# pengsongyou/openscene

Hardware: AMD Instinct MI355X
Metric: active voxels/sec MinkUNet18A fwd+bwd @2cm ScanNet; per-point query ms (higher is better)
Workload: dtype f32 (bf16x6 split-precision MFMA, fp32 accumulate); 1 GPU; ScanNet distillation step (configs[2]): MinkUNet18A, 768-d head, 1 synthetic S100k scene/GPU (100999 voxels on rank 0, 2 cm), training-mode BN; timed = coordinate+kernel maps, forward, cosine loss, backward, gradient all-reduce, Adam step; arch=MinkUNet18A, feature_dim=768, voxels_rank0=100999, parallelism=dp1

## Files before the change

### openscene_amd/csrc/bn.hip

```cpp
#include "common.h"
#include "epilogue.h"

namespace osn {

constexpr int CR_COLS = 64;
constexpr int CR_RL = 16;
constexpr int CR_MAX_BLOCKS = 512;

constexpr int BN_MAX_SRC = 3;
struct GySrc {
    const float* p[BN_MAX_SRC];
    int64_t ld[BN_MAX_SRC];
    int n;
};

__device__ inline float4 gy_load(const GySrc& s, int64_t r, int col) {
    float4 g = *reinterpret_cast<const float4*>(s.p[0] + r * s.ld[0] + col);
#pragma unroll
    for (int i = 1; i < BN_MAX_SRC; ++i)
        if (i < s.n) {
            const float4 v = *reinterpret_cast<const float4*>(s.p[i] + r * s.ld[i] + col);
            g.x += v.x; g.y += v.y; g.z += v.z; g.w += v.w;
        }
    return g;
}


struct ColReducePlan {
    int n_rb;
    int n_cg;
    int rows_per_block;
};

static ColReducePlan plan_colreduce(int64_t n, int c) {
    ColReducePlan p;
    p.n_cg = int(cdiv(c, CR_COLS));
    int64_t rb = cdiv(n, 4 * CR_RL);
    if (rb > CR_MAX_BLOCKS) rb = CR_MAX_BLOCKS;
    if (rb < 1) rb = 1;
    p.rows_per_block = int(cdiv(cdiv(n, rb), CR_RL) * CR_RL);
    p.n_rb = int(cdiv(n, p.rows_per_block));
    if (p.n_rb < 1) p.n_rb = 1;
    return p;
}

template <int MODE>
__global__ __launch_bounds__(256) void col_reduce_kernel(const float* __restrict__ x, const float* __restrict__ y,
                                                         const GySrc gy, const float* __restrict__ mean,
                                                         const float* __restrict__ var, float eps, int relu, int64_t n,
                                                         int c, int rows_per_block, double* __restrict__ partial,
                                                         const float* __restrict__ gamma, const float* __restrict__ beta) {
    __shared__ double red[2][CR_RL][CR_COLS];
    const int tid = threadIdx.x;
    const int cl = tid & 15, rl = tid >> 4;
    const int col = blockIdx.y * CR_COLS + cl * 4;
    const bool on = col < c;
    const int64_t r0 = int64_t(blockIdx.x) * rows_per_block;
    const int64_t r1 = min(n, r0 + rows_per_block);
    double s1[4] = {0, 0, 0, 0}, s2[4] = {0, 0, 0, 0};
    float4 mu = make_float4(0, 0, 0, 0), is = make_float4(0, 0, 0, 0);
    float4 ga = make_float4(0, 0, 0, 0), be = make_float4(0, 0, 0, 0);
    const bool from_x = MODE == 1 && relu && !y;
    if (MODE == 1 && on) {
        mu = *reinterpret_cast<const float4*>(mean + col);
        const float4 v = *reinterpret_cast<const float4*>(var + col);
        is = make_float4(bn_is(v.x, eps), bn_is(v.y, eps), bn_is(v.z, eps), bn_is(v.w, eps));
        if (from_x) {
            ga = *reinterpret_cast<const float4*>(gamma + col);
            be = *reinterpret_cast<const float4*>(beta + col);
        }
    }
    if (on) {
        for (int64_t r = r0 + rl; r < r1; r += CR_RL) {
            const float4 xv = *reinterpret_cast<const float4*>(x + r * c + col);
            if (MODE == 0) {
                s1[0] += xv.x; s1[1] += xv.y; s1[2] += xv.z; s1[3] += xv.w;
                s2[0] += double(xv.x) * xv.x; s2[1] += double(xv.y) * xv.y;
                s2[2] += double(xv.z) * xv.z; s2[3] += double(xv.w) * xv.w;
            } else {
                float4 g = gy_load(gy, r, col);
                if (from_x) {
                    g.x = bn_val(xv.x, mu.x, is.x, ga.x, be.x) > 0.f ? g.x : 0.f;
                    g.y = bn_val(xv.y, mu.y, is.y, ga.y, be.y) > 0.f ? g.y : 0.f;
                    g.z = bn_val(xv.z, mu.z, is.z, ga.z, be.z) > 0.f ? g.z : 0.f;
                    g.w = bn_val(xv.w, mu.w, is.w, ga.w, be.w) > 0.f ? g.w : 0.f;
                } else if (relu) {
                    const float4 yv = *reinterpret_cast<const float4*>(y + r * c + col);
                    g.x = yv.x > 0.f ? g.x : 0.f; g.y = yv.y > 0.f ? g.y : 0.f;
                    g.z = yv.z > 0.f ? g.z : 0.f; g.w = yv.w > 0.f ? g.w : 0.f;
                }
                s1[0] += g.x; s1[1] += g.y; s1[2] += g.z; s1[3] += g.w;
                s2[0] += double(g.x) * ((xv.x - mu.x) * is.x); s2[1] += double(g.y) * ((xv.y - mu.y) * is.y);
                s2[2] += double(g.z) * ((xv.z - mu.z) * is.z); s2[3] += double(g.w) * ((xv.w - mu.w) * is.w);
            }
        }
    }
#pragma unroll
    for (int j = 0; j < 4; ++j) {
        red[0][rl][cl * 4 + j] = s1[j];
        red[1][rl][cl * 4 + j] = s2[j];
    }
    __syncthreads();
    if (tid < 2 * CR_COLS) {
        const int which = tid / CR_COLS, cc = tid % CR_COLS;
        double s = 0;
#pragma unroll
        for (int r = 0; r < CR_RL; ++r) s += red[which][r][cc];
        const int gc = blockIdx.y * CR_COLS + cc;
        if (gc < c) partial[(int64_t(blockIdx.x) * 2 + which) * c + gc] = s;
    }
}

constexpr int FIN_COLS = 16, FIN_PARTS = 64;

constexpr int FIN_ITERS = CR_MAX_BLOCKS / FIN_PARTS;

__device__ inline void finalize_sums(const double* __restrict__ partial, int n_rb, int c, double& s1, double& s2,
                                     int& col) {
    __shared__ double red[2][FIN_PARTS][FIN_COLS];
    const int cl = threadIdx.x & (FIN_COLS - 1), part = threadIdx.x / FIN_COLS;
    col = blockIdx.x * FIN_COLS + cl;
    double va[FIN_ITERS], vb[FIN_ITERS];
    const int cc = col < c ? col : 0;
#pragma unroll
    for (int i = 0; i < FIN_ITERS; ++i) {
        const int blk = part + FIN_PARTS * i;
        const int bc = blk < n_rb ? blk : 0;
        va[i] = partial[(int64_t(bc) * 2 + 0) * c + cc];
        vb[i] = partial[(int64_t(bc) * 2 + 1) * c + cc];
    }
    double a = 0, b = 0;
#pragma unroll
    for (int i = 0; i < FIN_ITERS; ++i) {
        const bool on = col < c && part + FIN_PARTS * i < n_rb;
        a += on ? va[i] : 0.0;
        b += on ? vb[i] : 0.0;
    }
    red[0][part][cl] = a;
    red[1][part][cl] = b;
    __syncthreads();
    double t1 = 0, t2 = 0;
    if (part < 8) {
#pragma unroll
        for (int q = 0; q < 8; ++q) { t1 += red[0][part * 8 + q][cl]; t2 += red[1][part * 8 + q][cl]; }
    }
    __syncthreads();
    if (part < 8) {
        red[0][part][cl] = t1;
        red[1][part][cl] = t2;
    }
    __syncthreads();
    s1 = 0; s2 = 0;
    if (part == 0) {
#pragma unroll
        for (int q = 0; q < 8; ++q) { s1 += red[0][q][cl]; s2 += red[1][q][cl]; }
    }
}

__global__ __launch_bounds__(FIN_COLS * FIN_PARTS) void bn_stats_finalize_kernel(
    const double* __restrict__ partial, int n_rb, int64_t n, int c, float* __restrict__ mean, float* __restrict__ var,
    float* __restrict__ running_mean, float* __restrict__ running_var, float momentum) {
    double s1, s2;
    int j;
    finalize_sums(partial, n_rb, c, s1, s2, j);
    if (threadIdx.x >= FIN_COLS || j >= c) return;
    const double m = s1 / double(n);
    double v = s2 / double(n) - m * m;
    if (v < 0) v = 0;
    mean[j] = float(m);
    var[j] = float(v);
    if (running_mean) running_mean[j] = (1.f - momentum) * running_mean[j] + momentum * float(m);
    if (running_var) {
        const double unb = n > 1 ? v * double(n) / double(n - 1) : v;
        running_var[j] = (1.f - momentum) * running_var[j] + momentum * float(unb);
    }
}

__global__ __launch_bounds__(FIN_COLS * FIN_PARTS) void bn_bwd_finalize_kernel(const double* __restrict__ partial,
                                                                              int n_rb, int c,
                                                                              float* __restrict__ sum_g,
                                                                              float* __restrict__ sum_gx) {
    double s1, s2;
    int j;
    finalize_sums(partial, n_rb, c, s1, s2, j);
    if (threadIdx.x >= FIN_COLS || j >= c) return;
    sum_g[j] = float(s1);
    sum_gx[j] = float(s2);
}

__device__ inline float4 ld4(const float* p) { return *reinterpret_cast<const float4*>(p); }


__global__ __launch_bounds__(256) void bn_apply_kernel(const float* __restrict__ x, const float* __restrict__ mean,
                                                       const float* __restrict__ var, const float* __restrict__ gamma,
                                                       const float* __restrict__ beta, float eps,
                                                       const float* __restrict__ residual, int relu,
                                                       float* __restrict__ y, float* __restrict__ y2, int64_t ld2,
                                                       int64_t total4, int c4) {
    for (int64_t e = int64_t(blockIdx.x) * blockDim.x + threadIdx.x; e < total4; e += int64_t(gridDim.x) * blockDim.x) {
        const int col = int(e % c4) * 4;
        const float4 xv = ld4(x + e * 4), mu = ld4(mean + col), vv = ld4(var + col), ga = ld4(gamma + col),
                     be = ld4(beta + col);
        float4 o;
        o.x = bn_val(xv.x, mu.x, bn_is(vv.x, eps), ga.x, be.x);
        o.y = bn_val(xv.y, mu.y, bn_is(vv.y, eps), ga.y, be.y);
        o.z = bn_val(xv.z, mu.z, bn_is(vv.z, eps), ga.z, be.z);
        o.w = bn_val(xv.w, mu.w, bn_is(vv.w, eps), ga.w, be.w);
        if (residual) {
            const float4 rv = ld4(residual + e * 4);
            o.x += rv.x; o.y += rv.y; o.z += rv.z; o.w += rv.w;
        }
        if (relu) {
            o.x = bn_relu(o.x); o.y = bn_relu(o.y); o.z = bn_relu(o.z); o.w = bn_relu(o.w);
        }
        *reinterpret_cast<float4*>(y + e * 4) = o;
        if (y2) *reinterpret_cast<float4*>(y2 + (e / c4) * ld2 + col) = o;
    }
}

__global__ __launch_bounds__(256) void bn_bwd_apply_kernel(const float* __restrict__ x, const float* __restrict__ y,
                                                           const GySrc gy, const float* __restrict__ mean,
                                                           const float* __restrict__ var, const float* __restrict__ gamma,
                                                           float eps, int relu, int training,
                                                           const float* __restrict__ sum_g,
                                                           const float* __restrict__ sum_gx, float inv_n,
                                                           float* __restrict__ gx, float* __restrict__ gres,
                                                           int64_t total4, int c4, const float* __restrict__ beta) {
    const bool from_x = relu && !y;
    for (int64_t e = int64_t(blockIdx.x) * blockDim.x + threadIdx.x; e < total4; e += int64_t(gridDim.x) * blockDim.x) {
        const int col = int(e % c4) * 4;
        float4 g = gy_load(gy, e / c4, col);
        const float4 vv = ld4(var + col), ga = ld4(gamma + col);
        const float4 is = make_float4(bn_is(vv.x, eps), bn_is(vv.y, eps), bn_is(vv.z, eps), bn_is(vv.w, eps));
        float4 xv = make_float4(0, 0, 0, 0), mu = make_float4(0, 0, 0, 0);
        if (training || from_x) { xv = ld4(x + e * 4); mu = ld4(mean + col); }
        if (from_x) {
            const float4 be = ld4(beta + col);
            g.x = bn_val(xv.x, mu.x, is.x, ga.x, be.x) > 0.f ? g.x : 0.f;
            g.y = bn_val(xv.y, mu.y, is.y, ga.y, be.y) > 0.f ? g.y : 0.f;
            g.z = bn_val(xv.z, mu.z, is.z, ga.z, be.z) > 0.f ? g.z : 0.f;
            g.w = bn_val(xv.w, mu.w, is.w, ga.w, be.w) > 0.f ? g.w : 0.f;
        } else if (relu) {
            const float4 yv = ld4(y + e * 4);
            g.x = yv.x > 0.f ? g.x : 0.f; g.y = yv.y > 0.f ? g.y : 0.f;
            g.z = yv.z > 0.f ? g.z : 0.f; g.w = yv.w > 0.f ? g.w : 0.f;
        }
        if (gres) *reinterpret_cast<float4*>(gres + e * 4) = g;
        float4 o;
        if (training) {
            const float4 sg = ld4(sum_g + col), sx = ld4(sum_gx + col);
            o.x = ga.x * is.x * (g.x - sg.x * inv_n - (xv.x - mu.x) * is.x * sx.x * inv_n);
            o.y = ga.y * is.y * (g.y - sg.y * inv_n - (xv.y - mu.y) * is.y * sx.y * inv_n);
            o.z = ga.z * is.z * (g.z - sg.z * inv_n - (xv.z - mu.z) * is.z * sx.z * inv_n);
            o.w = ga.w * is.w * (g.w - sg.w * inv_n - (xv.w - mu.w) * is.w * sx.w * inv_n);
        } else {
            o.x = ga.x * is.x * g.x; o.y = ga.y * is.y * g.y; o.z = ga.z * is.z * g.z; o.w = ga.w * is.w * g.w;
        }
        *reinterpret_cast<float4*>(gx + e * 4) = o;
    }
}

constexpr int SB_THREADS = 1024, SB_RL = 512, SB_PER = 8, SB_COLS = 8;
constexpr int SB_MAX_ROWS = SB_RL * SB_PER;

__device__ inline double sb_wave_sum(double v) {
#pragma unroll
    for (int off = 2; off < 64; off <<= 1) v += __shfl_xor(v, off, 64);
    return v;
}

__device__ inline void sb_block_sums(double (&s)[8], int tid, int cl) {
    __shared__ double red[SB_THREADS / 64][2][8];
    __shared__ double tot[2][8];
#pragma unroll
    for (int q = 0; q < 8; ++q) s[q] = sb_wave_sum(s[q]);
    const int lane = tid & 63, wave = tid >> 6;
    if ((lane >> 1) == 0) {
#pragma unroll
        for (int q = 0; q < 8; ++q) red[wave][cl][q] = s[q];
    }
    __syncthreads();
    if (tid < 16) {
        const int c2 = tid >> 3, q = tid & 7;
        double t = 0;
#pragma unroll
        for (int w = 0; w < SB_THREADS / 64; ++w) t += red[w][c2][q];
        tot[c2][q] = t;
    }
    __syncthreads();
#pragma unroll
    for (int q = 0; q < 8; ++q) s[q] = tot[cl][q];
}

__global__ __launch_bounds__(SB_THREADS) void bn_small_fwd_kernel(const float* __restrict__ x, int n, int c,
                                                                  const float* __restrict__ gamma, const float* __restrict__ beta,
                                                                  float eps, const float* __restrict__ residual, int relu,
                                                                  float momentum, float* __restrict__ mean_out,
                                                                  float* __restrict__ var_out, float* __restrict__ running_mean,
                                                                  float* __restrict__ running_var, float* __restrict__ y,
                                                                  float* __restrict__ y2, int64_t ld2) {
    const int tid = threadIdx.x, cl = tid & 1, rl = tid >> 1;
    const int col = blockIdx.x * SB_COLS + cl * 4;
    const bool con = col < c;
    const int cc = con ? col : 0;
    float4 v[SB_PER];
    double s[8] = {0, 0, 0, 0, 0, 0, 0, 0};
#pragma unroll
    for (int j = 0; j < SB_PER; ++j) {
        const int r = rl + SB_RL * j;
        const bool ok = con && r < n;
        v[j] = ld4(x + int64_t(ok ? r : 0) * c + cc);
        if (ok) {
            s[0] += v[j].x; s[1] += v[j].y; s[2] += v[j].z; s[3] += v[j].w;
            s[4] += double(v[j].x) * v[j].x; s[5] += double(v[j].y) * v[j].y;
            s[6] += double(v[j].z) * v[j].z; s[7] += double(v[j].w) * v[j].w;
        }
    }
    sb_block_sums(s, tid, cl);
    float mu[4], vr[4];
#pragma unroll
    for (int q = 0; q < 4; ++q) {
        const double m = s[q] / double(n);
        double var = s[4 + q] / double(n) - m * m;
        if (var < 0) var = 0;
        mu[q] = float(m);
        vr[q] = float(var);
        if (rl == 0 && con) {
            mean_out[col + q] = mu[q];
            var_out[col + q] = vr[q];
            if (running_mean) running_mean[col + q] = (1.f - momentum) * running_mean[col + q] + momentum * mu[q];
            if (running_var) {
                const double unb = n > 1 ? var * double(n) / double(n - 1) : var;
                running_var[col + q] = (1.f - momentum) * running_var[col + q] + momentum * float(unb);
            }
        }
    }
    if (!con) return;
    const float4 ga = ld4(gamma + col), be = ld4(beta + col);
    const float is0 = bn_is(vr[0], eps), is1 = bn_is(vr[1], eps), is2 = bn_is(vr[2], eps), is3 = bn_is(vr[3], eps);
#pragma unroll
    for (int j = 0; j < SB_PER; ++j) {
        const int r = rl + SB_RL * j;
        if (r >= n) continue;
        float4 o;
        o.x = bn_val(v[j].x, mu[0], is0, ga.x, be.x);
        o.y = bn_val(v[j].y, mu[1], is1, ga.y, be.y);
        o.z = bn_val(v[j].z, mu[2], is2, ga.z, be.z);
        o.w = bn_val(v[j].w, mu[3], is3, ga.w, be.w);
        if (residual) {
            const float4 rv = ld4(residual + int64_t(r) * c + col);
            o.x += rv.x; o.y += rv.y; o.z += rv.z; o.w += rv.w;
        }
        if (relu) {
            o.x = bn_relu(o.x); o.y = bn_relu(o.y); o.z = bn_relu(o.z); o.w = bn_relu(o.w);
        }
        *reinterpret_cast<float4*>(y + int64_t(r) * c + col) = o;
        if (y2) *reinterpret_cast<float4*>(y2 + int64_t(r) * ld2 + col) = o;
    }
}

static int ew_grid(int64_t total4) {
    int64_t g = cdiv(total4, 256);
    if (g > 2048) g = 2048;
    if (g < 1) g = 1;
    return int(g);
}

}

using namespace osn;

extern "C" size_t osn_bn_ws_bytes(int64_t n, int c) {
    (void)n;
    return size_t(CR_MAX_BLOCKS) * 2 * size_t(c) * 8 + 256;
}

extern "C" int osn_bn_stats(const float* x, int64_t n, int c, float* mean, float* var, float* running_mean,
                            float* running_var, float momentum, void* ws, size_t ws_bytes, osn_stream_t stream) {
    hipStream_t st = static_cast<hipStream_t>(stream);
    OSN_REQUIRE(n >= 1 && c >= 4 && (c & 3) == 0, OSN_E_ARG, "osn_bn_stats: need n >= 1 and c %% 4 == 0 (n=%lld c=%d)", (long long)n, c);
    OSN_REQUIRE(x && mean && var && aligned16(x), OSN_E_ARG, "osn_bn_stats: null or unaligned pointer");
    ColReducePlan p = plan_colreduce(n, c);
    const size_t need = size_t(p.n_rb) * 2 * size_t(c) * 8;
    OSN_REQUIRE(ws && ws_bytes >= need, OSN_E_WS, "osn_bn_stats: workspace %zu < %zu", ws_bytes, need);
    double* partial = static_cast<double*>(ws);
    hipLaunchKernelGGL((col_reduce_kernel<0>), dim3(p.n_rb, p.n_cg), dim3(256), 0, st, x, (const float*)nullptr,
                       GySrc{}, (const float*)nullptr, (const float*)nullptr, 0.f, 0, n, c,
                       p.rows_per_block, partial, (const float*)nullptr, (const float*)nullptr);
    hipLaunchKernelGGL(bn_stats_finalize_kernel, dim3(cdiv(c, FIN_COLS)), dim3(FIN_COLS * FIN_PARTS), 0, st, partial, p.n_rb, n, c, mean, var,
                       running_mean, running_var, momentum);
    OSN_LAUNCH_CHECK();
    return OSN_OK;
}

extern "C" int osn_bn_apply2(const float* x, const float* mean, const float* var, const float* gamma, const float* beta,
                             float eps, const float* residual, int relu, float* y, float* y2, int64_t ld2, int64_t n, int c,
                             osn_stream_t stream) {
    hipStream_t st = static_cast<hipStream_t>(stream);
    OSN_REQUIRE(n >= 0 && c >= 4 && (c & 3) == 0, OSN_E_ARG, "osn_bn_apply: need c %% 4 == 0 (c=%d)", c);
    if (n == 0) return OSN_OK;
    OSN_REQUIRE(x && mean && var && gamma && beta && y, OSN_E_ARG, "osn_bn_apply: null pointer");
    OSN_REQUIRE(aligned16(x) && aligned16(y) && aligned16(mean) && aligned16(var) && aligned16(gamma) && aligned16(beta) &&
                    (!residual || aligned16(residual)),
                OSN_E_ARG, "osn_bn_apply: pointers must be 16-byte aligned");
    OSN_REQUIRE(!y2 || (aligned16(y2) && ld2 >= c && (ld2 & 3) == 0), OSN_E_ARG,
                "osn_bn_apply2: the second destination needs a 16-byte aligned pointer and a row stride >= c, %% 4 == 0");
    const int64_t total4 = n * (c / 4);
    hipLaunchKernelGGL(bn_apply_kernel, dim3(ew_grid(total4)), dim3(256), 0, st, x, mean, var, gamma, beta, eps,
                       residual, relu, y, y2, ld2, total4, c / 4);
    OSN_LAUNCH_CHECK();
    return OSN_OK;
}

extern "C" int osn_bn_apply(const float* x, const float* mean, const float* var, const float* gamma, const float* beta,
                            float eps, const float* residual, int relu, float* y, int64_t n, int c,
                            osn_stream_t stream) {
    return osn_bn_apply2(x, mean, var, gamma, beta, eps, residual, relu, y, nullptr, 0, n, c, stream);
}

extern "C" int osn_bn_forward_train2(const float* x, int64_t n, int c, const float* gamma, const float* beta, float eps,
                                     const float* residual, int relu, float momentum, float* mean, float* var,
                                     float* running_mean, float* running_var, float* y, float* y2, int64_t ld2, void* ws,
                                     size_t ws_bytes, osn_stream_t stream) {
    if (n >= 1 && n <= SB_MAX_ROWS && c >= 4 && (c & 3) == 0) {
        hipStream_t st = static_cast<hipStream_t>(stream);
        OSN_REQUIRE(x && mean && var && gamma && beta && y, OSN_E_ARG, "osn_bn_forward_train: null pointer");
        OSN_REQUIRE(aligned16(x) && aligned16(y) && aligned16(gamma) && aligned16(beta) && (!residual || aligned16(residual)),
                    OSN_E_ARG, "osn_bn_forward_train: pointers must be 16-byte aligned");
        OSN_REQUIRE(!y2 || (aligned16(y2) && ld2 >= c && (ld2 & 3) == 0), OSN_E_ARG,
                    "osn_bn_forward_train2: the second destination needs a 16-byte aligned pointer and a row stride >= c, %% 4 == 0");
        hipLaunchKernelGGL(bn_small_fwd_kernel, dim3(unsigned(cdiv(c, SB_COLS))), dim3(SB_THREADS), 0, st, x, int(n), c, gamma,
                           beta, eps, residual, relu, momentum, mean, var, running_mean, running_var, y, y2, ld2);
        OSN_LAUNCH_CHECK();
        return OSN_OK;
    }
    int rc = osn_bn_stats(x, n, c, mean, var, running_mean, running_var, momentum, ws, ws_bytes, stream);
    if (rc) return rc;
    return osn_bn_apply2(x, mean, var, gamma, beta, eps, residual, relu, y, y2, ld2, n, c, stream);
}

extern "C" int osn_bn_forward_train(const float* x, int64_t n, int c, const float* gamma, const float* beta, float eps,
                                    const float* residual, int relu, float momentum, float* mean, float* var,
                                    float* running_mean, float* running_var, float* y, void* ws, size_t ws_bytes,
                                    osn_stream_t stream) {
    return osn_bn_forward_train2(x, n, c, gamma, beta, eps, residual, relu, momentum, mean, var, running_mean, running_var, y,
                                 nullptr, 0, ws, ws_bytes, stream);
}

extern "C" int osn_bn_backward_multi2(const float* x, const float* y, const float* const* gy, const int64_t* gy_ld, int n_gy,
                                      const float* mean, const float* var, const float* gamma, const float* beta, float eps, int relu,
                                     int training, float* gx, float* gres, float* ggamma, float* gbeta, int64_t n, int c,
                                     void* ws, size_t ws_bytes, osn_stream_t stream) {
    hipStream_t st = static_cast<hipStream_t>(stream);
    OSN_REQUIRE(n >= 1 && c >= 4 && (c & 3) == 0, OSN_E_ARG, "osn_bn_backward: need n >= 1 and c %% 4 == 0");
    OSN_REQUIRE(gy && gy_ld && n_gy >= 1 && n_gy <= BN_MAX_SRC, OSN_E_ARG,
                "osn_bn_backward: %d gradient sources (1 .. %d are supported)", n_gy, BN_MAX_SRC);
    OSN_REQUIRE(x && mean && var && gamma && gx && ggamma && gbeta && (!relu || y || beta), OSN_E_ARG,
                "osn_bn_backward: null pointer");
    OSN_REQUIRE(!(relu && !y) || !gres, OSN_E_ARG, "osn_bn_backward: the ReLU mask can be recomputed from x only without a residual");
    OSN_REQUIRE(!beta || aligned16(beta), OSN_E_ARG, "osn_bn_backward: beta must be 16-byte aligned");
    OSN_REQUIRE(aligned16(x) && aligned16(gx) && aligned16(mean) && aligned16(var) && aligned16(gamma) &&
                    aligned16(ggamma) && aligned16(gbeta) && (!y || aligned16(y)) && (!gres || aligned16(gres)),
                OSN_E_ARG, "osn_bn_backward: pointers must be 16-byte aligned");
    GySrc src{};
    src.n = n_gy;
    for (int i = 0; i < BN_MAX_SRC; ++i) {
        const int j = i < n_gy ? i : 0;
        OSN_REQUIRE(gy[j] && aligned16(gy[j]) && gy_ld[j] >= c && (gy_ld[j] & 3) == 0, OSN_E_ARG,
                    "osn_bn_backward: gradient source %d needs a 16-byte aligned pointer and a row stride >= c, %% 4 == 0", j);
        src.p[i] = gy[j];
        src.ld[i] = gy_ld[j];
    }
    ColReducePlan p = plan_colreduce(n, c);
    const size_t need = size_t(p.n_rb) * 2 * size_t(c) * 8;
    OSN_REQUIRE(ws && ws_bytes >= need, OSN_E_WS, "osn_bn_backward: workspace %zu < %zu", ws_bytes, need);
    double* partial = static_cast<double*>(ws);
    hipLaunchKernelGGL((col_reduce_kernel<1>), dim3(p.n_rb, p.n_cg), dim3(256), 0, st, x, y, src, mean, var, eps, relu, n,
                       c, p.rows_per_block, partial, gamma, beta);
    hipLaunchKernelGGL(bn_bwd_finalize_kernel, dim3(cdiv(c, FIN_COLS)), dim3(FIN_COLS * FIN_PARTS), 0, st, partial, p.n_rb, c, gbeta, ggamma);
    const int64_t total4 = n * (c / 4);
    hipLaunchKernelGGL(bn_bwd_apply_kernel, dim3(ew_grid(total4)), dim3(256), 0, st, x, y, src, mean, var, gamma, eps,
                       relu, training, gbeta, ggamma, 1.f / float(n), gx, gres, total4, c / 4, beta);
    OSN_LAUNCH_CHECK();
    return OSN_OK;
}

extern "C" int osn_bn_backward_multi(const float* x, const float* y, const float* const* gy, const int64_t* gy_ld, int n_gy,
                                     const float* mean, const float* var, const float* gamma, float eps, int relu,
                                     int training, float* gx, float* gres, float* ggamma, float* gbeta, int64_t n, int c,
                                     void* ws, size_t ws_bytes, osn_stream_t stream) {
    OSN_REQUIRE(!relu || y, OSN_E_ARG, "osn_bn_backward_multi: relu needs y (or osn_bn_backward_multi2 with beta)");
    return osn_bn_backward_multi2(x, y, gy, gy_ld, n_gy, mean, var, gamma, nullptr, eps, relu, training, gx, gres, ggamma, gbeta, n, c,
                                  ws, ws_bytes, stream);
}

extern "C" int osn_bn_backward(const float* x, const float* y, const float* gy, const float* mean, const float* var,
                               const float* gamma, float eps, int relu, int training, float* gx, float* gres,
                               float* ggamma, float* gbeta, int64_t n, int c, void* ws, size_t ws_bytes,
                               osn_stream_t stream) {
    const int64_t ld = c;
    return osn_bn_backward_multi(x, y, &gy, &ld, 1, mean, var, gamma, eps, relu, training, gx, gres, ggamma, gbeta, n, c, ws,
                                 ws_bytes, stream);
}
```

Before: 12.38 million voxels/s.

## Restructure batch-norm column reductions and fuse finalize into apply kernels

Reworks the BN column-reduction kernels to use 512-thread blocks with adaptive column-lane width, unrolled row loads, and wave-shuffle reductions. For large inputs, the finalize step is folded into the forward and backward apply kernels: each block re-reduces the partial sums itself instead of a separate finalize launch. This cuts kernel launches and the single-block finalize serialization. The cost is redundant partial-sum reads per block and a more complex launch plan with two template variants.

```diff
diff --git a/openscene_amd/csrc/bn.hip b/openscene_amd/csrc/bn.hip
--- a/openscene_amd/csrc/bn.hip
+++ b/openscene_amd/csrc/bn.hip
@@ -3,9 +3,14 @@
 
 namespace osn {
 
-constexpr int CR_COLS = 64;
-constexpr int CR_RL = 16;
-constexpr int CR_MAX_BLOCKS = 512;
+constexpr int BN_T = 512;
+constexpr int BN_U = 4;
+constexpr int BN_MAX_RB = 256;
+constexpr int BN_WG_TARGET = 512;
+constexpr int FIN_PARTS = 16;
+constexpr int FIN_ITERS = BN_MAX_RB / FIN_PARTS;
+constexpr int SB_THREADS = 1024, SB_RL = 512, SB_PER = 8, SB_COLS = 8;
+constexpr int SB_MAX_ROWS = SB_RL * SB_PER;
 
 constexpr int BN_MAX_SRC = 3;
 struct GySrc {
@@ -26,42 +31,79 @@
 }
 
 
-struct ColReducePlan {
-    int n_rb;
-    int n_cg;
-    int rows_per_block;
+
+struct BnPlan {
+    int cl, n_cg, n_rb, rows_per_block;
+    bool fused_fwd, fused_bwd;
 };
 
-static ColReducePlan plan_colreduce(int64_t n, int c) {
-    ColReducePlan p;
-    p.n_cg = int(cdiv(c, CR_COLS));
-    int64_t rb = cdiv(n, 4 * CR_RL);
-    if (rb > CR_MAX_BLOCKS) rb = CR_MAX_BLOCKS;
+static BnPlan plan_bn(int64_t n, int c) {
+    BnPlan p;
+    const int c4 = c / 4;
+    p.cl = (c4 % 16 == 0) ? 16 : ((c4 % 8 == 0 || c4 <= 8) ? 8 : 16);
+    p.n_cg = int(cdiv(c4, p.cl));
+    const int rl = BN_T / p.cl;
+    int64_t rb = cdiv(n, int64_t(rl) * BN_U);
+    int64_t cap = BN_WG_TARGET / p.n_cg;
+    if (cap > BN_MAX_RB) cap = BN_MAX_RB;
+    if (cap < 1) cap = 1;
+    if (rb > cap) rb = cap;
     if (rb < 1) rb = 1;
-    p.rows_per_block = int(cdiv(cdiv(n, rb), CR_RL) * CR_RL);
+    p.rows_per_block = int(cdiv(cdiv(n, rb), rl) * rl);
     p.n_rb = int(cdiv(n, p.rows_per_block));
     if (p.n_rb < 1) p.n_rb = 1;
+    p.fused_fwd = n > SB_MAX_ROWS;
+    p.fused_bwd = n > SB_MAX_ROWS;
     return p;
 }
 
-template <int MODE>
-__global__ __launch_bounds__(256) void col_reduce_kernel(const float* __restrict__ x, const float* __restrict__ y,
-                                                         const GySrc gy, const float* __restrict__ mean,
-                                                         const float* __restrict__ var, float eps, int relu, int64_t n,
-                                                         int c, int rows_per_block, double* __restrict__ partial,
-                                                         const float* __restrict__ gamma, const float* __restrict__ beta) {
-    __shared__ double red[2][CR_RL][CR_COLS];
-    const int tid = threadIdx.x;
-    const int cl = tid & 15, rl = tid >> 4;
-    const int col = blockIdx.y * CR_COLS + cl * 4;
-    const bool on = col < c;
+template <int CL>
+struct BnLanes {
+    static constexpr int WRL = 64 / CL, RL = (BN_T / 64) * WRL, CT = CL * 4;
+    int cl, rl, col;
+    bool on;
+    __device__ BnLanes(int c) {
+        const int lane = threadIdx.x & 63, wave = threadIdx.x >> 6;
+        cl = lane % CL;
+        rl = wave * WRL + lane / CL;
+        col = blockIdx.y * CT + cl * 4;
+        on = col < c;
+    }
+};
+
+__device__ inline float4 bn_masked(float4 g, const float4 xv, const float4 yv, bool from_x, bool relu, const float4 mu,
+                                   const float4 is, const float4 ga, const float4 be) {
+    if (from_x) {
+        g.x = bn_val(xv.x, mu.x, is.x, ga.x, be.x) > 0.f ? g.x : 0.f;
+        g.y = bn_val(xv.y, mu.y, is.y, ga.y, be.y) > 0.f ? g.y : 0.f;
+        g.z = bn_val(xv.z, mu.z, is.z, ga.z, be.z) > 0.f ? g.z : 0.f;
+        g.w = bn_val(xv.w, mu.w, is.w, ga.w, be.w) > 0.f ? g.w : 0.f;
+    } else if (relu) {
+        g.x = yv.x > 0.f ? g.x : 0.f; g.y = yv.y > 0.f ? g.y : 0.f;
+        g.z = yv.z > 0.f ? g.z : 0.f; g.w = yv.w > 0.f ? g.w : 0.f;
+    }
+    return g;
+}
+
+template <int MODE, int CL>
+__global__ __launch_bounds__(BN_T) void col_reduce_kernel(const float* __restrict__ x, const float* __restrict__ y,
+                                                          const GySrc gy, const float* __restrict__ mean,
+                                                          const float* __restrict__ var, float eps, int relu, int64_t n,
+                                                          int c, int rows_per_block, double* __restrict__ partial,
+                                                          const float* __restrict__ gamma, const float* __restrict__ beta) {
+    using L = BnLanes<CL>;
+    constexpr int NW = BN_T / 64;
+    __shared__ double red[NW][2][L::CT];
+    const L t(c);
+    const int col = t.col;
     const int64_t r0 = int64_t(blockIdx.x) * rows_per_block;
     const int64_t r1 = min(n, r0 + rows_per_block);
-    double s1[4] = {0, 0, 0, 0}, s2[4] = {0, 0, 0, 0};
+    double s[8] = {0, 0, 0, 0, 0, 0, 0, 0};
     float4 mu = make_float4(0, 0, 0, 0), is = make_float4(0, 0, 0, 0);
     float4 ga = make_float4(0, 0, 0, 0), be = make_float4(0, 0, 0, 0);
     const bool from_x = MODE == 1 && relu && !y;
-    if (MODE == 1 && on) {
+    const bool from_y = MODE == 1 && relu && y;
+    if (MODE == 1 && t.on) {
         mu = *reinterpret_cast<const float4*>(mean + col);
         const float4 v = *reinterpret_cast<const float4*>(var + col);
         is = make_float4(bn_is(v.x, eps), bn_is(v.y, eps), bn_is(v.z, eps), bn_is(v.w, eps));
@@ -70,126 +112,162 @@
             be = *reinterpret_cast<const float4*>(beta + col);
         }
     }
-    if (on) {
-        for (int64_t r = r0 + rl; r < r1; r += CR_RL) {
-            const float4 xv = *reinterpret_cast<const float4*>(x + r * c + col);
-            if (MODE == 0) {
-                s1[0] += xv.x; s1[1] += xv.y; s1[2] += xv.z; s1[3] += xv.w;
-                s2[0] += double(xv.x) * xv.x; s2[1] += double(xv.y) * xv.y;
-                s2[2] += double(xv.z) * xv.z; s2[3] += double(xv.w) * xv.w;
-            } else {
-                float4 g = gy_load(gy, r, col);
-                if (from_x) {
-                    g.x = bn_val(xv.x, mu.x, is.x, ga.x, be.x) > 0.f ? g.x : 0.f;
-                    g.y = bn_val(xv.y, mu.y, is.y, ga.y, be.y) > 0.f ? g.y : 0.f;
-                    g.z = bn_val(xv.z, mu.z, is.z, ga.z, be.z) > 0.f ? g.z : 0.f;
-                    g.w = bn_val(xv.w, mu.w, is.w, ga.w, be.w) > 0.f ? g.w : 0.f;
-                } else if (relu) {
-                    const float4 yv = *reinterpret_cast<const float4*>(y + r * c + col);
-                    g.x = yv.x > 0.f ? g.x : 0.f; g.y = yv.y > 0.f ? g.y : 0.f;
-                    g.z = yv.z > 0.f ? g.z : 0.f; g.w = yv.w > 0.f ? g.w : 0.f;
+    if (t.on) {
+        for (int64_t rb = r0 + t.rl; rb < r1; rb += int64_t(L::RL) * BN_U) {
+            float4 xv[BN_U], g[BN_U], yv[BN_U];
+#pragma unroll
+            for (int u = 0; u < BN_U; ++u) {
+                const int64_t r = rb + u * L::RL < r1 ? rb + u * L::RL : rb;
+                xv[u] = *reinterpret_cast<const float4*>(x + r * c + col);
+                if (MODE == 1) {
+                    g[u] = gy_load(gy, r, col);
+                    yv[u] = from_y ? *reinterpret_cast<const float4*>(y + r * c + col) : make_float4(0, 0, 0, 0);
                 }
-                s1[0] += g.x; s1[1] += g.y; s1[2] += g.z; s1[3] += g.w;
-                s2[0] += double(g.x) * ((xv.x - mu.x) * is.x); s2[1] += double(g.y) * ((xv.y - mu.y) * is.y);
-                s2[2] += double(g.z) * ((xv.z - mu.z) * is.z); s2[3] += double(g.w) * ((xv.w - mu.w) * is.w);
             }
-        }
-    }
-#pragma unroll
-    for (int j = 0; j < 4; ++j) {
-        red[0][rl][cl * 4 + j] = s1[j];
-        red[1][rl][cl * 4 + j] = s2[j];
+#pragma unroll
+            for (int u = 0; u < BN_U; ++u) {
+                if (rb + u * L::RL >= r1) break;
+                const float4 xu = xv[u];
+                if (MODE == 0) {
+                    s[0] += xu.x; s[1] += xu.y; s[2] += xu.z; s[3] += xu.w;
+                    s[4] += double(xu.x) * xu.x; s[5] += double(xu.y) * xu.y;
+                    s[6] += double(xu.z) * xu.z; s[7] += double(xu.w) * xu.w;
+                } else {
+                    const float4 gu = bn_masked(g[u], xu, yv[u], from_x, relu, mu, is, ga, be);
+                    s[0] += gu.x; s[1] += gu.y; s[2] += gu.z; s[3] += gu.w;
+                    s[4] += double(gu.x) * ((xu.x - mu.x) * is.x); s[5] += double(gu.y) * ((xu.y - mu.y) * is.y);
+                    s[6] += double(gu.z) * ((xu.z - mu.z) * is.z); s[7] += double(gu.w) * ((xu.w - mu.w) * is.w);
+                }
+            }
+        }
+    }
+#pragma unroll
+    for (int off = CL; off < 64; off <<= 1) {
+#pragma unroll
+        for (int q = 0; q < 8; ++q) s[q] += __shfl_xor(s[q], off, 64);
+    }
+    const int lane = threadIdx.x & 63, wave = threadIdx.x >> 6;
+    if (lane < CL) {
+#pragma unroll
+        for (int j = 0; j < 4; ++j) {
+            red[wave][0][t.cl * 4 + j] = s[j];
+            red[wave][1][t.cl * 4 + j] = s[4 + j];
+        }
     }
     __syncthreads();
-    if (tid < 2 * CR_COLS) {
-        const int which = tid / CR_COLS, cc = tid % CR_COLS;
-        double s = 0;
-#pragma unroll
-        for (int r = 0; r < CR_RL; ++r) s += red[which][r][cc];
-        const int gc = blockIdx.y * CR_COLS + cc;
-        if (gc < c) partial[(int64_t(blockIdx.x) * 2 + which) * c + gc] = s;
-    }
-}
-
-constexpr int FIN_COLS = 16, FIN_PARTS = 64;
-
-constexpr int FIN_ITERS = CR_MAX_BLOCKS / FIN_PARTS;
-
-__device__ inline void finalize_sums(const double* __restrict__ partial, int n_rb, int c, double& s1, double& s2,
-                                     int& col) {
-    __shared__ double red[2][FIN_PARTS][FIN_COLS];
-    const int cl = threadIdx.x & (FIN_COLS - 1), part = threadIdx.x / FIN_COLS;
-    col = blockIdx.x * FIN_COLS + cl;
-    double va[FIN_ITERS], vb[FIN_ITERS];
-    const int cc = col < c ? col : 0;
-#pragma unroll
-    for (int i = 0; i < FIN_ITERS; ++i) {
-        const int blk = part + FIN_PARTS * i;
-        const int bc = blk < n_rb ? blk : 0;
-        va[i] = partial[(int64_t(bc) * 2 + 0) * c + cc];
-        vb[i] = partial[(int64_t(bc) * 2 + 1) * c + cc];
-    }
-    double a = 0, b = 0;
-#pragma unroll
-    for (int i = 0; i < FIN_ITERS; ++i) {
-        const bool on = col < c && part + FIN_PARTS * i < n_rb;
-        a += on ? va[i] : 0.0;
-        b += on ? vb[i] : 0.0;
-    }
-    red[0][part][cl] = a;
-    red[1][part][cl] = b;
+    if (threadIdx.x < 2 * L::CT) {
+        const int which = threadIdx.x / L::CT, cc = threadIdx.x % L::CT;
+        double a = 0;
+#pragma unroll
+        for (int w = 0; w < NW; ++w) a += red[w][which][cc];
+        const int gc = blockIdx.y * L::CT + cc;
+        if (gc < c) partial[(int64_t(blockIdx.x) * 2 + which) * c + gc] = a;
+    }
+}
+
+template <int CT>
+__device__ inline bool bn_column_sums(const double* __restrict__ partial, int n_rb, int c, int col0, double& s1, double& s2,
+                                      int& col) {
+    __shared__ double chain[2][FIN_PARTS][CT];
+    for (int w = threadIdx.x; w < 2 * FIN_PARTS * CT; w += BN_T) {
+        const int cc = w % CT, part = (w / CT) % FIN_PARTS, which = w / (CT * FIN_PARTS);
+        const int gc = col0 + cc < c ? col0 + cc : 0;
+        double v[FIN_ITERS];
+#pragma unroll
+        for (int i = 0; i < FIN_ITERS; ++i) {
+            const int blk = part + FIN_PARTS * i;
+            v[i] = partial[(int64_t(blk < n_rb ? blk : 0) * 2 + which) * c + gc];
+        }
+        double a = 0;
+#pragma unroll
+        for (int i = 0; i < FIN_ITERS; ++i) a += part + FIN_PARTS * i < n_rb ? v[i] : 0.0;
+        chain[which][part][cc] = a;
+    }
     __syncthreads();
-    double t1 = 0, t2 = 0;
-    if (part < 8) {
-#pragma unroll
-        for (int q = 0; q < 8; ++q) { t1 += red[0][part * 8 + q][cl]; t2 += red[1][part * 8 + q][cl]; }
-    }
-    __syncthreads();
-    if (part < 8) {
-        red[0][part][cl] = t1;
-        red[1][part][cl] = t2;
-    }
-    __syncthreads();
+    col = col0 + int(threadIdx.x);
     s1 = 0; s2 = 0;
-    if (part == 0) {
-#pragma unroll
-        for (int q = 0; q < 8; ++q) { s1 += red[0][q][cl]; s2 += red[1][q][cl]; }
-    }
-}
-
-__global__ __launch_bounds__(FIN_COLS * FIN_PARTS) void bn_stats_finalize_kernel(
+    if (threadIdx.x >= CT || col >= c) return false;
+#pragma unroll
+    for (int q = 0; q < FIN_PARTS; ++q) { s1 += chain[0][q][threadIdx.x]; s2 += chain[1][q][threadIdx.x]; }
+    return true;
+}
+
+__device__ inline void bn_stats_of_sums(double s1, double s2, int64_t n, int j, bool write, float* __restrict__ mean,
+                                        float* __restrict__ var, float* __restrict__ running_mean,
+                                        float* __restrict__ running_var, float momentum, float& mu, float& vr) {
+    const double m = s1 / double(n);
+    double v = s2 / double(n) - m * m;
+    if (v < 0) v = 0;
+    mu = float(m);
+    vr = float(v);
+    if (!write) return;
+    mean[j] = mu;
+    var[j] = vr;
+    if (running_mean) running_mean[j] = (1.f - momentum) * running_mean[j] + momentum * float(m);
+    if (running_var) {
+        const double unb = n > 1 ? v * double(n) / double(n - 1) : v;
+        running_var[j] = (1.f - momentum) * running_var[j] + momentum * float(unb);
+    }
+}
+
+template <int CL>
+__global__ __launch_bounds__(BN_T) void bn_stats_finalize_kernel(
     const double* __restrict__ partial, int n_rb, int64_t n, int c, float* __restrict__ mean, float* __restrict__ var,
     float* __restrict__ running_mean, float* __restrict__ running_var, float momentum) {
     double s1, s2;
     int j;
-    finalize_sums(partial, n_rb, c, s1, s2, j);
-    if (threadIdx.x >= FIN_COLS || j >= c) return;
-    const double m = s1 / double(n);
-    double v = s2 / double(n) - m * m;
-    if (v < 0) v = 0;
-    mean[j] = float(m);
-    var[j] = float(v);
-    if (running_mean) running_mean[j] = (1.f - momentum) * running_mean[j] + momentum * float(m);
-    if (running_var) {
-        const double unb = n > 1 ? v * double(n) / double(n - 1) : v;
-        running_var[j] = (1.f - momentum) * running_var[j] + momentum * float(unb);
-    }
-}
-
-__global__ __launch_bounds__(FIN_COLS * FIN_PARTS) void bn_bwd_finalize_kernel(const double* __restrict__ partial,
-                                                                              int n_rb, int c,
-                                                                              float* __restrict__ sum_g,
-                                                                              float* __restrict__ sum_gx) {
+    if (!bn_column_sums<CL * 4>(partial, n_rb, c, blockIdx.x * CL * 4, s1, s2, j)) return;
+    float mu, vr;
+    bn_stats_of_sums(s1, s2, n, j, true, mean, var, running_mean, running_var, momentum, mu, vr);
+}
+
+template <int CL>
+__global__ __launch_bounds__(BN_T) void bn_bwd_finalize_kernel(const double* __restrict__ partial, int n_rb, int c,
+                                                               float* __restrict__ sum_g, float* __restrict__ sum_gx) {
     double s1, s2;
     int j;
-    finalize_sums(partial, n_rb, c, s1, s2, j);
-    if (threadIdx.x >= FIN_COLS || j >= c) return;
+    if (!bn_column_sums<CL * 4>(partial, n_rb, c, blockIdx.x * CL * 4, s1, s2, j)) return;
     sum_g[j] = float(s1);
     sum_gx[j] = float(s2);
 }
 
 __device__ inline float4 ld4(const float* p) { return *reinterpret_cast<const float4*>(p); }
 
+
+__device__ inline float4 bn_fwd4(const float4 xv, const float4 mu, const float4 is, const float4 ga, const float4 be,
+                                 const float* __restrict__ res, int relu) {
+    float4 o;
+    o.x = bn_val(xv.x, mu.x, is.x, ga.x, be.x);
+    o.y = bn_val(xv.y, mu.y, is.y, ga.y, be.y);
+    o.z = bn_val(xv.z, mu.z, is.z, ga.z, be.z);
+    o.w = bn_val(xv.w, mu.w, is.w, ga.w, be.w);
+    if (res) {
+        const float4 rv = ld4(res);
+        o.x += rv.x; o.y += rv.y; o.z += rv.z; o.w += rv.w;
+    }
+    if (relu) {
+        o.x = bn_relu(o.x); o.y = bn_relu(o.y); o.z = bn_relu(o.z); o.w = bn_relu(o.w);
+    }
+    return o;
+}
+
+__device__ inline float4 bn_bwd4(const float4 g, const float4 xv, const float4 mu, const float4 is, const float4 ga,
+                                 const float4 sg, const float4 sx, float inv_n, int training) {
+    float4 o;
+    if (training) {
+        o.x = ga.x * is.x * (g.x - sg.x * inv_n - (xv.x - mu.x) * is.x * sx.x * inv_n);
+        o.y = ga.y * is.y * (g.y - sg.y * inv_n - (xv.y - mu.y) * is.y * sx.y * inv_n);
+        o.z = ga.z * is.z * (g.z - sg.z * inv_n - (xv.z - mu.z) * is.z * sx.z * inv_n);
+        o.w = ga.w * is.w * (g.w - sg.w * inv_n - (xv.w - mu.w) * is.w * sx.w * inv_n);
+    } else {
+        o.x = ga.x * is.x * g.x; o.y = ga.y * is.y * g.y; o.z = ga.z * is.z * g.z; o.w = ga.w * is.w * g.w;
+    }
+    return o;
+}
+
+__device__ inline float4 bn_is4(const float4 vv, float eps) {
+    return make_float4(bn_is(vv.x, eps), bn_is(vv.y, eps), bn_is(vv.z, eps), bn_is(vv.w, eps));
+}
 
 __global__ __launch_bounds__(256) void bn_apply_kernel(const float* __restrict__ x, const float* __restrict__ mean,
                                                        const float* __restrict__ var, const float* __restrict__ gamma,
@@ -201,18 +279,7 @@
         const int col = int(e % c4) * 4;
         const float4 xv = ld4(x + e * 4), mu = ld4(mean + col), vv = ld4(var + col), ga = ld4(gamma + col),
                      be = ld4(beta + col);
-        float4 o;
-        o.x = bn_val(xv.x, mu.x, bn_is(vv.x, eps), ga.x, be.x);
-        o.y = bn_val(xv.y, mu.y, bn_is(vv.y, eps), ga.y, be.y);
-        o.z = bn_val(xv.z, mu.z, bn_is(vv.z, eps), ga.z, be.z);
-        o.w = bn_val(xv.w, mu.w, bn_is(vv.w, eps), ga.w, be.w);
-        if (residual) {
-            const float4 rv = ld4(residual + e * 4);
-            o.x += rv.x; o.y += rv.y; o.z += rv.z; o.w += rv.w;
-        }
-        if (relu) {
-            o.x = bn_relu(o.x); o.y = bn_relu(o.y); o.z = bn_relu(o.z); o.w = bn_relu(o.w);
-        }
+        const float4 o = bn_fwd4(xv, mu, bn_is4(vv, eps), ga, be, residual ? residual + e * 4 : nullptr, relu);
         *reinterpret_cast<float4*>(y + e * 4) = o;
         if (y2) *reinterpret_cast<float4*>(y2 + (e / c4) * ld2 + col) = o;
     }
@@ -227,41 +294,121 @@
                                                            float* __restrict__ gx, float* __restrict__ gres,
                                                            int64_t total4, int c4, const float* __restrict__ beta) {
     const bool from_x = relu && !y;
+    const float4 z4 = make_float4(0, 0, 0, 0);
     for (int64_t e = int64_t(blockIdx.x) * blockDim.x + threadIdx.x; e < total4; e += int64_t(gridDim.x) * blockDim.x) {
         const int col = int(e % c4) * 4;
         float4 g = gy_load(gy, e / c4, col);
         const float4 vv = ld4(var + col), ga = ld4(gamma + col);
-        const float4 is = make_float4(bn_is(vv.x, eps), bn_is(vv.y, eps), bn_is(vv.z, eps), bn_is(vv.w, eps));
-        float4 xv = make_float4(0, 0, 0, 0), mu = make_float4(0, 0, 0, 0);
+        const float4 is = bn_is4(vv, eps);
+        float4 xv = z4, mu = z4;
         if (training || from_x) { xv = ld4(x + e * 4); mu = ld4(mean + col); }
-        if (from_x) {
-            const float4 be = ld4(beta + col);
-            g.x = bn_val(xv.x, mu.x, is.x, ga.x, be.x) > 0.f ? g.x : 0.f;
-            g.y = bn_val(xv.y, mu.y, is.y, ga.y, be.y) > 0.f ? g.y : 0.f;
-            g.z = bn_val(xv.z, mu.z, is.z, ga.z, be.z) > 0.f ? g.z : 0.f;
-            g.w = bn_val(xv.w, mu.w, is.w, ga.w, be.w) > 0.f ? g.w : 0.f;
-        } else if (relu) {
-            const float4 yv = ld4(y + e * 4);
-            g.x = yv.x > 0.f ? g.x : 0.f; g.y = yv.y > 0.f ? g.y : 0.f;
-            g.z = yv.z > 0.f ? g.z : 0.f; g.w = yv.w > 0.f ? g.w : 0.f;
-        }
+        g = bn_masked(g, xv, (relu && y) ? ld4(y + e * 4) : z4, from_x, relu, mu, is, ga, from_x ? ld4(beta + col) : z4);
         if (gres) *reinterpret_cast<float4*>(gres + e * 4) = g;
-        float4 o;
-        if (training) {
-            const float4 sg = ld4(sum_g + col), sx = ld4(sum_gx + col);
-            o.x = ga.x * is.x * (g.x - sg.x * inv_n - (xv.x - mu.x) * is.x * sx.x * inv_n);
-            o.y = ga.y * is.y * (g.y - sg.y * inv_n - (xv.y - mu.y) * is.y * sx.y * inv_n);
-            o.z = ga.z * is.z * (g.z - sg.z * inv_n - (xv.z - mu.z) * is.z * sx.z * inv_n);
-            o.w = ga.w * is.w * (g.w - sg.w * inv_n - (xv.w - mu.w) * is.w * sx.w * inv_n);
-        } else {
-            o.x = ga.x * is.x * g.x; o.y = ga.y * is.y * g.y; o.z = ga.z * is.z * g.z; o.w = ga.w * is.w * g.w;
-        }
-        *reinterpret_cast<float4*>(gx + e * 4) = o;
-    }
-}
-
-constexpr int SB_THREADS = 1024, SB_RL = 512, SB_PER = 8, SB_COLS = 8;
-constexpr int SB_MAX_ROWS = SB_RL * SB_PER;
+        const float4 sg = training ? ld4(sum_g + col) : z4, sx = training ? ld4(sum_gx + col) : z4;
+        *reinterpret_cast<float4*>(gx + e * 4) = bn_bwd4(g, xv, mu, is, ga, sg, sx, inv_n, training);
+    }
+}
+
+constexpr int BN_UA = 2;
+
+template <int CL>
+__global__ __launch_bounds__(BN_T) void bn_fwd_fused_kernel(const float* __restrict__ x, const double* __restrict__ partial,
+                                                            int n_rb, int64_t n, int c, int rows_per_block,
+                                                            const float* __restrict__ gamma, const float* __restrict__ beta,
+                                                            float eps, const float* __restrict__ residual, int relu,
+                                                            float momentum, float* __restrict__ mean, float* __restrict__ var,
+                                                            float* __restrict__ running_mean, float* __restrict__ running_var,
+                                                            float* __restrict__ y, float* __restrict__ y2, int64_t ld2) {
+    using L = BnLanes<CL>;
+    __shared__ __attribute__((aligned(16))) float fin[2][L::CT];
+    double s1, s2;
+    int j;
+    if (bn_column_sums<L::CT>(partial, n_rb, c, blockIdx.y * L::CT, s1, s2, j)) {
+        float mu, vr;
+        bn_stats_of_sums(s1, s2, n, j, blockIdx.x == 0, mean, var, running_mean, running_var, momentum, mu, vr);
+        fin[0][threadIdx.x] = mu;
+        fin[1][threadIdx.x] = vr;
+    }
+    __syncthreads();
+    const L t(c);
+    if (!t.on) return;
+    const int col = t.col;
+    const float4 mu = ld4(&fin[0][t.cl * 4]), is = bn_is4(ld4(&fin[1][t.cl * 4]), eps);
+    const float4 ga = ld4(gamma + col), be = ld4(beta + col);
+    const int64_t r0 = int64_t(blockIdx.x) * rows_per_block;
+    const int64_t r1 = min(n, r0 + rows_per_block);
+    for (int64_t rb = r0 + t.rl; rb < r1; rb += int64_t(L::RL) * BN_UA) {
+        float4 xv[BN_UA];
+#pragma unroll
+        for (int u = 0; u < BN_UA; ++u) {
+            const int64_t r = rb + u * L::RL < r1 ? rb + u * L::RL : rb;
+            xv[u] = ld4(x + r * c + col);
+        }
+#pragma unroll
+        for (int u = 0; u < BN_UA; ++u) {
+            const int64_t r = rb + u * L::RL;
+            if (r >= r1) break;
+            const float4 o = bn_fwd4(xv[u], mu, is, ga, be, residual ? residual + r * c + col : nullptr, relu);
+            *reinterpret_cast<float4*>(y + r * c + col) = o;
+            if (y2) *reinterpret_cast<float4*>(y2 + r * ld2 + col) = o;
+        }
+    }
+}
+
+template <int CL>
+__global__ __launch_bounds__(BN_T) void bn_bwd_fused_kernel(const float* __restrict__ x, const float* __restrict__ y,
+                                                            const GySrc gy, const double* __restrict__ partial, int n_rb,
+                                                            int64_t n, int c, int rows_per_block,
+                                                            const float* __restrict__ mean, const float* __restrict__ var,
+                                                            const float* __restrict__ gamma, const float* __restrict__ beta,
+                                                            float eps, int relu, int training, float inv_n,
+                                                            float* __restrict__ gx, float* __restrict__ gres,
+                                                            float* __restrict__ ggamma, float* __restrict__ gbeta) {
+    using L = BnLanes<CL>;
+    __shared__ __attribute__((aligned(16))) float fin[2][L::CT];
+    double s1, s2;
+    int j;
+    if (bn_column_sums<L::CT>(partial, n_rb, c, blockIdx.y * L::CT, s1, s2, j)) {
+        fin[0][threadIdx.x] = float(s1);
+        fin[1][threadIdx.x] = float(s2);
+        if (blockIdx.x == 0) {
+            gbeta[j] = float(s1);
+            ggamma[j] = float(s2);
+        }
+    }
+    __syncthreads();
+    const L t(c);
+    if (!t.on) return;
+    const int col = t.col;
+    const bool from_x = relu && !y;
+    const bool from_y = relu && y;
+    const bool need_x = training || from_x;
+    const float4 z4 = make_float4(0, 0, 0, 0);
+    const float4 sg = ld4(&fin[0][t.cl * 4]), sx = ld4(&fin[1][t.cl * 4]);
+    const float4 mu = ld4(mean + col), is = bn_is4(ld4(var + col), eps), ga = ld4(gamma + col);
+    const float4 be = from_x ? ld4(beta + col) : z4;
+    const int64_t r0 = int64_t(blockIdx.x) * rows_per_block;
+    const int64_t r1 = min(n, r0 + rows_per_block);
+    for (int64_t rb = r0 + t.rl; rb < r1; rb += int64_t(L::RL) * BN_UA) {
+        float4 xv[BN_UA], g[BN_UA], yv[BN_UA];
+#pragma unroll
+        for (int u = 0; u < BN_UA; ++u) {
+            const int64_t r = rb + u * L::RL < r1 ? rb + u * L::RL : rb;
+            g[u] = gy_load(gy, r, col);
+            xv[u] = need_x ? ld4(x + r * c + col) : z4;
+            yv[u] = from_y ? ld4(y + r * c + col) : z4;
+        }
+#pragma unroll
+        for (int u = 0; u < BN_UA; ++u) {
+            const int64_t r = rb + u * L::RL;
+            if (r >= r1) break;
+            const float4 gm = bn_masked(g[u], xv[u], yv[u], from_x, relu, mu, is, ga, be);
+            if (gres) *reinterpret_cast<float4*>(gres + r * c + col) = gm;
+            *reinterpret_cast<float4*>(gx + r * c + col) = bn_bwd4(gm, xv[u], mu, is, ga, sg, sx, inv_n, training);
+        }
+    }
+}
+
 
 __device__ inline double sb_wave_sum(double v) {
 #pragma unroll
@@ -372,7 +519,24 @@
 
 extern "C" size_t osn_bn_ws_bytes(int64_t n, int c) {
     (void)n;
-    return size_t(CR_MAX_BLOCKS) * 2 * size_t(c) * 8 + 256;
+    return size_t(BN_MAX_RB) * 2 * size_t(c) * 8 + 256;
+}
+
+static int bn_launch_stats_sums(const float* x, int64_t n, int c, const BnPlan& p, void* ws, size_t ws_bytes, hipStream_t st,
+                                double** partial) {
+    const size_t need = size_t(p.n_rb) * 2 * size_t(c) * 8;
+    OSN_REQUIRE(ws && ws_bytes >= need, OSN_E_WS, "osn_bn_stats: workspace %zu < %zu", ws_bytes, need);
+    *partial = static_cast<double*>(ws);
+    const dim3 grid(p.n_rb, p.n_cg);
+    if (p.cl == 8)
+        hipLaunchKernelGGL((col_reduce_kernel<0, 8>), grid, dim3(BN_T), 0, st, x, (const float*)nullptr, GySrc{},
+                           (const float*)nullptr, (const float*)nullptr, 0.f, 0, n, c, p.rows_per_block, *partial,
+                           (const float*)nullptr, (const float*)nullptr);
+    else
+        hipLaunchKernelGGL((col_reduce_kernel<0, 16>), grid, dim3(BN_T), 0, st, x, (const float*)nullptr, GySrc{},
+                           (const float*)nullptr, (const float*)nullptr, 0.f, 0, n, c, p.rows_per_block, *partial,
+                           (const float*)nullptr, (const float*)nullptr);
+    return OSN_OK;
 }
 
 extern "C" int osn_bn_stats(const float* x, int64_t n, int c, float* mean, float* var, float* running_mean,
@@ -380,15 +544,16 @@
     hipStream_t st = static_cast<hipStream_t>(stream);
     OSN_REQUIRE(n >= 1 && c >= 4 && (c & 3) == 0, OSN_E_ARG, "osn_bn_stats: need n >= 1 and c %% 4 == 0 (n=%lld c=%d)", (long long)n, c);
     OSN_REQUIRE(x && mean && var && aligned16(x), OSN_E_ARG, "osn_bn_stats: null or unaligned pointer");
-    ColReducePlan p = plan_colreduce(n, c);
-    const size_t need = size_t(p.n_rb) * 2 * size_t(c) * 8;
-    OSN_REQUIRE(ws && ws_bytes >= need, OSN_E_WS, "osn_bn_stats: workspace %zu < %zu", ws_bytes, need);
-    double* partial = static_cast<double*>(ws);
-    hipLaunchKernelGGL((col_reduce_kernel<0>), dim3(p.n_rb, p.n_cg), dim3(256), 0, st, x, (const float*)nullptr,
-                       GySrc{}, (const float*)nullptr, (const float*)nullptr, 0.f, 0, n, c,
-                       p.rows_per_block, partial, (const float*)nullptr, (const float*)nullptr);
-    hipLaunchKernelGGL(bn_stats_finalize_kernel, dim3(cdiv(c, FIN_COLS)), dim3(FIN_COLS * FIN_PARTS), 0, st, partial, p.n_rb, n, c, mean, var,
-                       running_mean, running_var, momentum);
+    const BnPlan p = plan_bn(n, c);
+    double* partial;
+    int rc = bn_launch_stats_sums(x, n, c, p, ws, ws_bytes, st, &partial);
+    if (rc) return rc;
+    if (p.cl == 8)
+        hipLaunchKernelGGL((bn_stats_finalize_kernel<8>), dim3(p.n_cg), dim3(BN_T), 0, st, partial, p.n_rb, n, c, mean, var,
+                           running_mean, running_var, momentum);
+    else
+        hipLaunchKernelGGL((bn_stats_finalize_kernel<16>), dim3(p.n_cg), dim3(BN_T), 0, st, partial, p.n_rb, n, c, mean, var,
+                           running_mean, running_var, momentum);
     OSN_LAUNCH_CHECK();
     return OSN_OK;
 }
@@ -431,6 +596,27 @@
                     "osn_bn_forward_train2: the second destination needs a 16-byte aligned pointer and a row stride >= c, %% 4 == 0");
         hipLaunchKernelGGL(bn_small_fwd_kernel, dim3(unsigned(cdiv(c, SB_COLS))), dim3(SB_THREADS), 0, st, x, int(n), c, gamma,
                            beta, eps, residual, relu, momentum, mean, var, running_mean, running_var, y, y2, ld2);
+        OSN_LAUNCH_CHECK();
+        return OSN_OK;
+    }
+    if (n > SB_MAX_ROWS && c >= 4 && (c & 3) == 0 && plan_bn(n, c).fused_fwd) {
+        hipStream_t st = static_cast<hipStream_t>(stream);
+        OSN_REQUIRE(x && mean && var && gamma && beta && y, OSN_E_ARG, "osn_bn_forward_train: null pointer");
+        OSN_REQUIRE(aligned16(x) && aligned16(y) && aligned16(gamma) && aligned16(beta) && (!residual || aligned16(residual)),
+                    OSN_E_ARG, "osn_bn_forward_train: pointers must be 16-byte aligned");
+        OSN_REQUIRE(!y2 || (aligned16(y2) && ld2 >= c && (ld2 & 3) == 0), OSN_E_ARG,
+                    "osn_bn_forward_train2: the second destination needs a 16-byte aligned pointer and a row stride >= c, %% 4 == 0");
+        const BnPlan p = plan_bn(n, c);
+        double* partial;
+        int rc = bn_launch_stats_sums(x, n, c, p, ws, ws_bytes, st, &partial);
+        if (rc) return rc;
+        const dim3 grid(p.n_rb, p.n_cg);
+        if (p.cl == 8)
+            hipLaunchKernelGGL((bn_fwd_fused_kernel<8>), grid, dim3(BN_T), 0, st, x, partial, p.n_rb, n, c, p.rows_per_block, gamma,
+                               beta, eps, residual, relu, momentum, mean, var, running_mean, running_var, y, y2, ld2);
+        else
+            hipLaunchKernelGGL((bn_fwd_fused_kernel<16>), grid, dim3(BN_T), 0, st, x, partial, p.n_rb, n, c, p.rows_per_block, gamma,
+                               beta, eps, residual, relu, momentum, mean, var, running_mean, running_var, y, y2, ld2);
         OSN_LAUNCH_CHECK();
         return OSN_OK;
     }
@@ -471,16 +657,35 @@
         src.p[i] = gy[j];
         src.ld[i] = gy_ld[j];
     }
-    ColReducePlan p = plan_colreduce(n, c);
+    const BnPlan p = plan_bn(n, c);
     const size_t need = size_t(p.n_rb) * 2 * size_t(c) * 8;
     OSN_REQUIRE(ws && ws_bytes >= need, OSN_E_WS, "osn_bn_backward: workspace %zu < %zu", ws_bytes, need);
     double* partial = static_cast<double*>(ws);
-    hipLaunchKernelGGL((col_reduce_kernel<1>), dim3(p.n_rb, p.n_cg), dim3(256), 0, st, x, y, src, mean, var, eps, relu, n,
-                       c, p.rows_per_block, partial, gamma, beta);
-    hipLaunchKernelGGL(bn_bwd_finalize_kernel, dim3(cdiv(c, FIN_COLS)), dim3(FIN_COLS * FIN_PARTS), 0, st, partial, p.n_rb, c, gbeta, ggamma);
+    const dim3 grid(p.n_rb, p.n_cg);
+    const float inv_n = 1.f / float(n);
+    if (p.cl == 8)
+        hipLaunchKernelGGL((col_reduce_kernel<1, 8>), grid, dim3(BN_T), 0, st, x, y, src, mean, var, eps, relu, n, c,
+                           p.rows_per_block, partial, gamma, beta);
+    else
+        hipLaunchKernelGGL((col_reduce_kernel<1, 16>), grid, dim3(BN_T), 0, st, x, y, src, mean, var, eps, relu, n, c,
+                           p.rows_per_block, partial, gamma, beta);
+    if (p.fused_bwd) {
+        if (p.cl == 8)
+            hipLaunchKernelGGL((bn_bwd_fused_kernel<8>), grid, dim3(BN_T), 0, st, x, y, src, partial, p.n_rb, n, c,
+                               p.rows_per_block, mean, var, gamma, beta, eps, relu, training, inv_n, gx, gres, ggamma, gbeta);
+        else
+            hipLaunchKernelGGL((bn_bwd_fused_kernel<16>), grid, dim3(BN_T), 0, st, x, y, src, partial, p.n_rb, n, c,
+                               p.rows_per_block, mean, var, gamma, beta, eps, relu, training, inv_n, gx, gres, ggamma, gbeta);
+        OSN_LAUNCH_CHECK();
+        return OSN_OK;
+    }
+    if (p.cl == 8)
+        hipLaunchKernelGGL((bn_bwd_finalize_kernel<8>), dim3(p.n_cg), dim3(BN_T), 0, st, partial, p.n_rb, c, gbeta, ggamma);
+    else
+        hipLaunchKernelGGL((bn_bwd_finalize_kernel<16>), dim3(p.n_cg), dim3(BN_T), 0, st, partial, p.n_rb, c, gbeta, ggamma);
     const int64_t total4 = n * (c / 4);
     hipLaunchKernelGGL(bn_bwd_apply_kernel, dim3(ew_grid(total4)), dim3(256), 0, st, x, y, src, mean, var, gamma, eps,
-                       relu, training, gbeta, ggamma, 1.f / float(n), gx, gres, total4, c / 4, beta);
+                       relu, training, gbeta, ggamma, inv_n, gx, gres, total4, c / 4, beta);
     OSN_LAUNCH_CHECK();
     return OSN_OK;
 }
```

Result: no change. 12.29 million voxels/s (-0.7%).
